# ingonyama-zk/icicle-snark

Measured on AMD Instinct MI355X. Metric: groth16_prove_constraints_per_s, higher is better.
Workload: dtype u256 mod p (MSM: 9x29-bit limbs in u32, Montgomery R=2^261, lazy reduction; NTT: 9x29-bit limbs, lazy; QAP/vec ops: 8xu32 limbs, Montgomery R=2^256)

## Files before the change

### icicle-snark_amd/csrc/ntt.hip

```cpp
#include <atomic>
#include <mutex>
#include <string.h>
#include <vector>

#include "common.h"
#include "ff.h"
#include "fr29.h"
#include "ntt_fuse.h"

using namespace bn254;
using namespace isnark;

namespace {

constexpr int LOG_TILE = 11;
constexpr int NT = 256;
constexpr int MAX_LOG_R = 9;
constexpr int OMEGAS_COUNT = 28;

const uint32_t ROU28[8] = {0x725b19f0, 0x9bd61b6e, 0x41112ed4, 0x402d111e, 0x8ef62abc, 0x00e0a7eb, 0xa58a7e85, 0x2a3c09f0};

struct Domain {
  fe* tw = nullptr;
  fe* tw29 = nullptr;
  int log_n = -1;
  fe root_std;
  int device = -1;
};
constexpr int MAX_DEVICES = 32;
std::mutex g_dom_mu;
Domain g_doms[MAX_DEVICES];
Domain& cur_dom()
{
  int d = 0;
  if (hipGetDevice(&d) != hipSuccess || d < 0 || d >= MAX_DEVICES) d = 0;
  return g_doms[d];
}
#define g_dom cur_dom()

fe host_omega(int logn)
{
  fe w;
  memcpy(w.l, ROU28, 32);
  w = Fr::to_mont(w);
  for (int i = 0; i < OMEGAS_COUNT - logn; i++) w = Fr::sqr(w);
  return Fr::from_mont(w);
}

__global__ void gen_twiddles_kernel(fe* tw, const fe* pw , int log_n)
{
  uint32_t i = blockIdx.x * blockDim.x + threadIdx.x;
  if (i >= (1u << log_n)) return;
  fe acc = Fr::one_mont();
  for (int j = 0; j < log_n; j++)
    if ((i >> j) & 1) acc = Fr::mul(acc, pw[j]);
  tw[i] = acc;
}

struct PassParams {
  int log_r, log_c;
  uint32_t tiles_per_group_log;
  uint64_t in_hi, in_lo, in_row, in_col;
  uint64_t out_hi, out_lo, out_row, out_col;
  uint32_t tw_mul;
  uint32_t stage_stride;
  uint32_t n_mask;
  int inverse;
  int scale;
  uint64_t batch_stride;
  int load_rows_fastest;
  const fe* scale_tab;
  uint32_t scale_stride;
  int fuse_abc;
  uint32_t xcd_batch;
};

__device__ __forceinline__ uint32_t tw_index(uint32_t e, uint32_t n_mask, int inverse)
{
  return inverse ? ((n_mask + 1 - e) & n_mask) : e;
}

__device__ __forceinline__ fe lds_get(const uint4* lo, const uint4* hi, int idx)
{
  uint4 a = lo[idx], b = hi[idx];
  fe r;
  r.l[0] = a.x; r.l[1] = a.y; r.l[2] = a.z; r.l[3] = a.w;
  r.l[4] = b.x; r.l[5] = b.y; r.l[6] = b.z; r.l[7] = b.w;
  return r;
}
__device__ __forceinline__ void lds_put(uint4* lo, uint4* hi, int idx, const fe& v)
{
  lo[idx] = make_uint4(v.l[0], v.l[1], v.l[2], v.l[3]);
  hi[idx] = make_uint4(v.l[4], v.l[5], v.l[6], v.l[7]);
}
__device__ __forceinline__ fe g_get(const fe* p)
{
  const uint4* q = reinterpret_cast<const uint4*>(p);
  uint4 a = q[0], b = q[1];
  fe r;
  r.l[0] = a.x; r.l[1] = a.y; r.l[2] = a.z; r.l[3] = a.w;
  r.l[4] = b.x; r.l[5] = b.y; r.l[6] = b.z; r.l[7] = b.w;
  return r;
}
__device__ __forceinline__ void g_put(fe* p, const fe& v)
{
  uint4* q = reinterpret_cast<uint4*>(p);
  q[0] = make_uint4(v.l[0], v.l[1], v.l[2], v.l[3]);
  q[1] = make_uint4(v.l[4], v.l[5], v.l[6], v.l[7]);
}

#define NTT_BF(a, b, e)                                                                                        \
  {                                                                                                            \
    const fe s_ = Fr::add(x[a], x[b]);                                                                         \
    const fe d_ = Fr::sub(x[a], x[b]);                                                                         \
    x[a] = s_;                                                                                                 \
    x[b] = Fr::mul(d_, lds_get(twlo, twhi, (e)));                                                              \
  }
template <int Q>
__device__ __forceinline__ void dif_butterfly(fe (&x)[1 << Q], int j, int log_m, int log_r, const uint4* twlo, const uint4* twhi);

template <>
__device__ __forceinline__ void dif_butterfly<3>(fe (&x)[8], int j, int log_m, int log_r, const uint4* twlo, const uint4* twhi)
{
  const int g = 1 << (log_m - 3);
  const int s0 = log_r - log_m, s1 = s0 + 1, s2 = s0 + 2;
  NTT_BF(0, 4, j << s0) NTT_BF(1, 5, (j + g) << s0) NTT_BF(2, 6, (j + 2 * g) << s0) NTT_BF(3, 7, (j + 3 * g) << s0)
  NTT_BF(0, 2, j << s1) NTT_BF(1, 3, (j + g) << s1) NTT_BF(4, 6, j << s1) NTT_BF(5, 7, (j + g) << s1)
  NTT_BF(0, 1, j << s2) NTT_BF(2, 3, j << s2) NTT_BF(4, 5, j << s2) NTT_BF(6, 7, j << s2)
}
template <>
__device__ __forceinline__ void dif_butterfly<2>(fe (&x)[4], int j, int log_m, int log_r, const uint4* twlo, const uint4* twhi)
{
  const int g = 1 << (log_m - 2);
  const int s0 = log_r - log_m, s1 = s0 + 1;
  NTT_BF(0, 2, j << s0) NTT_BF(1, 3, (j + g) << s0)
  NTT_BF(0, 1, j << s1) NTT_BF(2, 3, j << s1)
}
template <>
__device__ __forceinline__ void dif_butterfly<1>(fe (&x)[2], int j, int log_m, int log_r, const uint4* twlo, const uint4* twhi)
{
  NTT_BF(0, 1, j << (log_r - log_m))
}
#define NTT_BF1(a, b)                                                                                          \
  {                                                                                                            \
    const fe s_ = Fr::add(x[a], x[b]);                                                                         \
    x[b] = Fr::sub(x[a], x[b]);                                                                                \
    x[a] = s_;                                                                                                 \
  }
template <int Q>
__device__ __forceinline__ void dif_butterfly_last(fe (&x)[1 << Q], int log_r, const uint4* twlo, const uint4* twhi);
template <>
__device__ __forceinline__ void dif_butterfly_last<3>(fe (&x)[8], int log_r, const uint4* twlo, const uint4* twhi)
{
  const int s0 = log_r - 3, s1 = s0 + 1;
  NTT_BF1(0, 4) NTT_BF(1, 5, 1 << s0) NTT_BF(2, 6, 2 << s0) NTT_BF(3, 7, 3 << s0)
  NTT_BF1(0, 2) NTT_BF(1, 3, 1 << s1) NTT_BF1(4, 6) NTT_BF(5, 7, 1 << s1)
  NTT_BF1(0, 1) NTT_BF1(2, 3) NTT_BF1(4, 5) NTT_BF1(6, 7)
}
template <>
__device__ __forceinline__ void dif_butterfly_last<2>(fe (&x)[4], int log_r, const uint4* twlo, const uint4* twhi)
{
  const int s0 = log_r - 2;
  NTT_BF1(0, 2) NTT_BF(1, 3, 1 << s0)
  NTT_BF1(0, 1) NTT_BF1(2, 3)
}
template <>
__device__ __forceinline__ void dif_butterfly_last<1>(fe (&x)[2], int log_r, const uint4* twlo, const uint4* twhi)
{
  NTT_BF1(0, 1)
}
#undef NTT_BF1
#undef NTT_BF

template <int Q, bool LAST = false>
__device__ __forceinline__ void dif_round(uint4* lo, uint4* hi, const uint4* twlo, const uint4* twhi, int log_m, int log_r, int log_c, int tid)
{
  const int C = 1 << log_c;
  const int log_g = log_m - Q;
#pragma unroll
  for (int u = 0; u < (8 >> Q); u++) {
    const int gi = tid * (8 >> Q) + u;
    const int c = gi & (C - 1);
    const int rest = gi >> log_c;
    const int j = rest & ((1 << log_g) - 1);
    const int blk = rest >> log_g;
    const int base_row = (blk << log_m) + j;
    fe x[1 << Q];
#pragma unroll
    for (int k = 0; k < (1 << Q); k++) x[k] = lds_get(lo, hi, ((base_row + (k << log_g)) << log_c) + c);
    if (LAST) dif_butterfly_last<Q>(x, log_r, twlo, twhi);
    else dif_butterfly<Q>(x, j, log_m, log_r, twlo, twhi);
#pragma unroll
    for (int k = 0; k < (1 << Q); k++) lds_put(lo, hi, ((base_row + (k << log_g)) << log_c) + c, x[k]);
  }
}

template <int MODE>
__device__ __forceinline__ void ntt_tile_row(const fe* __restrict__ src, fe* __restrict__ dst, const fe* __restrict__ tw, const PassParams& p, const fe& ninv_mont, uint4* lo, uint4* hi,
                                             const uint4* twlo, const uint4* twhi, uint32_t b_lo, uint64_t out_off, int tid)
{
  const int R = 1 << p.log_r, C = 1 << p.log_c, RC = R * C;
  if (RC == NT * 8) {
    fe v[8];
#pragma unroll
    for (int u = 0; u < 8; u++) {
      const int e = tid + u * NT;
      int r, c;
      if (p.load_rows_fastest) { r = e & (R - 1); c = e >> p.log_r; }
      else { c = e & (C - 1); r = e >> p.log_c; }
      v[u] = g_get(src + (uint64_t)r * p.in_row + (uint64_t)c * p.in_col);
    }
#pragma unroll
    for (int u = 0; u < 8; u++) {
      const int e = tid + u * NT;
      int r, c;
      if (p.load_rows_fastest) { r = e & (R - 1); c = e >> p.log_r; }
      else { c = e & (C - 1); r = e >> p.log_c; }
      lds_put(lo, hi, (r << p.log_c) + c, v[u]);
    }
  } else {
    for (int e = tid; e < RC; e += NT) {
      int r, c;
      if (p.load_rows_fastest) { r = e & (R - 1); c = e >> p.log_r; }
      else { c = e & (C - 1); r = e >> p.log_c; }
      lds_put(lo, hi, (r << p.log_c) + c, g_get(src + (uint64_t)r * p.in_row + (uint64_t)c * p.in_col));
    }
  }
  __syncthreads();

  if (RC == NT * 8) {
    int log_m = p.log_r;
    while (log_m > 3) {
      dif_round<3>(lo, hi, twlo, twhi, log_m, p.log_r, p.log_c, tid);
      __syncthreads();
      log_m -= 3;
    }
    if (log_m == 3) dif_round<3, true>(lo, hi, twlo, twhi, log_m, p.log_r, p.log_c, tid);
    else if (log_m == 2) dif_round<2, true>(lo, hi, twlo, twhi, log_m, p.log_r, p.log_c, tid);
    else if (log_m == 1) dif_round<1, true>(lo, hi, twlo, twhi, log_m, p.log_r, p.log_c, tid);
    __syncthreads();
  } else {
    const int nbf = RC >> 1;
    for (int s = p.log_r - 1; s >= 0; s--) {
      const int h = 1 << s;
      for (int q = tid; q < nbf; q += NT) {
        const int c = q & (C - 1);
        const int bf = q >> p.log_c;
        const int j = bf & (h - 1);
        const int i = ((bf >> s) << (s + 1)) + j;
        const int ia = (i << p.log_c) + c, ib = ((i + h) << p.log_c) + c;
        fe a = lds_get(lo, hi, ia), bb = lds_get(lo, hi, ib);
        fe sum = Fr::add(a, bb);
        fe dif = Fr::sub(a, bb);
        const int e = j << (p.log_r - 1 - s);
        if (e != 0) dif = Fr::mul(dif, lds_get(twlo, twhi, e));
        lds_put(lo, hi, ia, sum);
        lds_put(lo, hi, ib, dif);
      }
      __syncthreads();
    }
  }

  if (MODE != 0) {
#pragma unroll 1
    for (int u0 = 0; u0 < 8; u0 += 4) {
      fe y[4];
      fe* q[4];
#pragma unroll
      for (int u = 0; u < 4; u++) {
        const int e = tid + (u0 + u) * NT;
        const int c = e & (C - 1);
        const uint32_t kk = __brev((uint32_t)(e >> p.log_c)) >> (32 - p.log_r);
        q[u] = dst + (uint64_t)kk * p.out_row + (uint64_t)c * p.out_col;
        if (MODE != 1) y[u] = g_get(q[u]);
      }
#pragma unroll
      for (int u = 0; u < 4; u++) {
        const fe x = lds_get(lo, hi, tid + (u0 + u) * NT);
        if (MODE == 1) g_put(q[u], x);
        else if (MODE == 2) g_put(q[u], Fr::mul(Fr::mul(x, y[u]), Fr::r2()));
        else g_put(q[u], Fr::sub(y[u], x));
      }
    }
    return;
  }
  for (int e0 = tid; e0 < RC; e0 += NT * 4) {
    fe w[4];
    uint32_t kk[4], ex[4];
#pragma unroll
    for (int u = 0; u < 4; u++) {
      const int e = e0 + u * NT;
      ex[u] = 0;
      if (e < RC) {
        const int c = e & (C - 1);
        kk[u] = __brev((uint32_t)(e >> p.log_c)) >> (32 - p.log_r);
        if (p.tw_mul) ex[u] = kk[u] * ((b_lo << p.log_c) + c) * p.tw_mul;
        if (ex[u]) w[u] = g_get(tw + tw_index(ex[u], p.n_mask, p.inverse));
      }
    }
#pragma unroll
    for (int u = 0; u < 4; u++) {
      const int e = e0 + u * NT;
      if (e < RC) {
        const int c = e & (C - 1);
        fe x = lds_get(lo, hi, e);
        if (ex[u]) x = Fr::mul(x, w[u]);
        if (p.scale_tab) x = Fr::mul(x, g_get(p.scale_tab + (out_off + (uint64_t)kk[u] * p.out_row + (uint64_t)c * p.out_col) * p.scale_stride));
        else if (p.scale) x = Fr::mul(x, ninv_mont);
        g_put(dst + (uint64_t)kk[u] * p.out_row + (uint64_t)c * p.out_col, x);
      }
    }
  }
}

template <bool FUSE>
__global__ __launch_bounds__(NT, 2) void ntt_pass_kernel(const fe* __restrict__ in, fe* __restrict__ out, const fe* __restrict__ tw, PassParams p, fe ninv_mont)
{
  ISNARK_CRITICAL_CHAIN_KERNEL();
  extern __shared__ __attribute__((aligned(16))) unsigned char smem[];
  const int R = 1 << p.log_r, C = 1 << p.log_c, RC = R * C;
  uint4* lo = reinterpret_cast<uint4*>(smem);
  uint4* hi = lo + RC;
  uint4* twlo = hi + RC;
  uint4* twhi = twlo + (R >> 1);

  const uint32_t b = blockIdx.x;
  const uint32_t b_hi = b >> p.tiles_per_group_log, b_lo = b & ((1u << p.tiles_per_group_log) - 1);
  const uint64_t in_off = b_hi * p.in_hi + b_lo * p.in_lo, out_off = b_hi * p.out_hi + b_lo * p.out_lo;
  const int tid = threadIdx.x;

  for (int e = tid; e < (R >> 1); e += NT) {
    fe w = g_get(tw + tw_index((uint32_t)e * p.stage_stride, p.n_mask, p.inverse));
    lds_put(twlo, twhi, e, w);
  }
  if (!FUSE) {
    ntt_tile_row<0>(in + (uint64_t)blockIdx.y * p.batch_stride + in_off, out + (uint64_t)blockIdx.y * p.batch_stride + out_off, tw, p, ninv_mont, lo, hi, twlo, twhi, b_lo, out_off, tid);
  } else {
    ntt_tile_row<1>(in + in_off, out + out_off, tw, p, ninv_mont, lo, hi, twlo, twhi, b_lo, out_off, tid);
    __syncthreads();
    ntt_tile_row<2>(in + p.batch_stride + in_off, out + out_off, tw, p, ninv_mont, lo, hi, twlo, twhi, b_lo, out_off, tid);
    __syncthreads();
    ntt_tile_row<3>(in + 2 * p.batch_stride + in_off, out + out_off, tw, p, ninv_mont, lo, hi, twlo, twhi, b_lo, out_off, tid);
  }
}

struct Plan29 {
  uint32_t b0;
  uint32_t bs;
  int shrink_last;
};
struct Lds29 {
  uint4 *lo, *hi;
  uint32_t* top;
};
__device__ __forceinline__ fe9 lds_get9(const Lds29& t, int idx)
{
  const uint4 a = t.lo[idx], b = t.hi[idx];
  fe9 r;
  r.l[0] = a.x; r.l[1] = a.y; r.l[2] = a.z; r.l[3] = a.w;
  r.l[4] = b.x; r.l[5] = b.y; r.l[6] = b.z; r.l[7] = b.w;
  r.l[8] = t.top[idx];
  return r;
}
__device__ __forceinline__ void lds_put9(const Lds29& t, int idx, const fe9& v)
{
  t.lo[idx] = make_uint4(v.l[0], v.l[1], v.l[2], v.l[3]);
  t.hi[idx] = make_uint4(v.l[4], v.l[5], v.l[6], v.l[7]);
  t.top[idx] = v.l[8];
}
__device__ __forceinline__ fe9 sub_k(const fe9& a, const fe9& b, const fr29::Limbs9& kc)
{
  fe9 o;
#pragma unroll
  for (int i = 0; i < 9; i++) o.l[i] = a.l[i] + (kc.v[i] - b.l[i]);
  return o;
}
#define NTT_BF9(a, b, e, NORM)                                                                                 \
  {                                                                                                            \
    const fe9 s_ = NORM ? fr29::norm(fr29::add(x[a], x[b])) : fr29::add(x[a], x[b]);                           \
    const fe9 d_ = sub_k(x[a], x[b], kc);                                                                      \
    x[a] = s_;                                                                                                 \
    x[b] = fr29::mul(d_, lds_get9(tw, (e)));                                                                   \
  }
#define NTT_BF9_1(a, b, NORM)                                                                                  \
  {                                                                                                            \
    const fe9 s_ = NORM ? fr29::norm(fr29::add(x[a], x[b])) : fr29::add(x[a], x[b]);                           \
    x[b] = fr29::norm(sub_k(x[a], x[b], kc));                                                                  \
    x[a] = s_;                                                                                                 \
  }
__device__ __forceinline__ uint32_t k_mid(const Plan29& pl, int l) { return (pl.b0 << l) + 1u; }
__device__ __forceinline__ uint32_t k_last(const Plan29& pl, int t) { return (pl.bs + 1u) << t; }

__device__ __forceinline__ void dif_butterfly9_mid(fe9 (&x)[8], int j, int log_m, int log_r, const Lds29& tw, const Plan29& pl)
{
  const int g = 1 << (log_m - 3);
  const int s0 = log_r - log_m, s1 = s0 + 1, s2 = s0 + 2;
  {
    const fr29::Limbs9 kc = fr29::kr_borrow_proof(k_mid(pl, s0), 1);
    NTT_BF9(0, 4, j << s0, false) NTT_BF9(1, 5, (j + g) << s0, false) NTT_BF9(2, 6, (j + 2 * g) << s0, false) NTT_BF9(3, 7, (j + 3 * g) << s0, false)
  }
  {
    const fr29::Limbs9 kc = fr29::kr_borrow_proof(k_mid(pl, s1), 2);
    NTT_BF9(0, 2, j << s1, true) NTT_BF9(1, 3, (j + g) << s1, true) NTT_BF9(4, 6, j << s1, true) NTT_BF9(5, 7, (j + g) << s1, true)
  }
  {
    const fr29::Limbs9 kc = fr29::kr_borrow_proof(k_mid(pl, s2), 1);
    NTT_BF9(0, 1, j << s2, true) NTT_BF9(2, 3, j << s2, true) NTT_BF9(4, 5, j << s2, true) NTT_BF9(6, 7, j << s2, true)
  }
}
template <int Q>
__device__ __forceinline__ void dif_butterfly9_last(fe9 (&x)[1 << Q], int log_r, const Lds29& tw, const Plan29& pl);
template <>
__device__ __forceinline__ void dif_butterfly9_last<3>(fe9 (&x)[8], int log_r, const Lds29& tw, const Plan29& pl)
{
  const int s0 = log_r - 3, s1 = s0 + 1;
  {
    const fr29::Limbs9 kc = fr29::kr_borrow_proof(k_last(pl, 0), 1);
    NTT_BF9_1(0, 4, false) NTT_BF9(1, 5, 1 << s0, false) NTT_BF9(2, 6, 2 << s0, false) NTT_BF9(3, 7, 3 << s0, false)
  }
  {
    const fr29::Limbs9 kc = fr29::kr_borrow_proof(k_last(pl, 1), 2);
    NTT_BF9_1(0, 2, true) NTT_BF9(1, 3, 1 << s1, true) NTT_BF9_1(4, 6, true) NTT_BF9(5, 7, 1 << s1, true)
  }
  {
    const fr29::Limbs9 kc = fr29::kr_borrow_proof(k_last(pl, 2), 1);
    NTT_BF9_1(0, 1, true) NTT_BF9_1(2, 3, true) NTT_BF9_1(4, 5, true) NTT_BF9_1(6, 7, true)
  }
}
template <>
__device__ __forceinline__ void dif_butterfly9_last<2>(fe9 (&x)[4], int log_r, const Lds29& tw, const Plan29& pl)
{
  const int s0 = log_r - 2;
  {
    const fr29::Limbs9 kc = fr29::kr_borrow_proof(k_last(pl, 0), 1);
    NTT_BF9_1(0, 2, false) NTT_BF9(1, 3, 1 << s0, false)
  }
  {
    const fr29::Limbs9 kc = fr29::kr_borrow_proof(k_last(pl, 1), 2);
    NTT_BF9_1(0, 1, true) NTT_BF9_1(2, 3, true)
  }
}
template <>
__device__ __forceinline__ void dif_butterfly9_last<1>(fe9 (&x)[2], int log_r, const Lds29& tw, const Plan29& pl)
{
  const fr29::Limbs9 kc = fr29::kr_borrow_proof(k_last(pl, 0), 1);
  NTT_BF9_1(0, 1, true)
}
#undef NTT_BF9_1
#undef NTT_BF9

template <int Q, bool LAST>
__device__ __forceinline__ void dif_round9(const Lds29& t, const Lds29& tw, int log_m, int log_r, int log_c, int tid, const Plan29& pl)
{
  const int C = 1 << log_c;
  const int log_g = log_m - Q;
#pragma unroll
  for (int u = 0; u < (8 >> Q); u++) {
    const int gi = tid * (8 >> Q) + u;
    const int c = gi & (C - 1);
    const int rest = gi >> log_c;
    const int j = rest & ((1 << log_g) - 1);
    const int blk = rest >> log_g;
    const int base_row = (blk << log_m) + j;
    fe9 x[1 << Q];
#pragma unroll
    for (int k = 0; k < (1 << Q); k++) x[k] = lds_get9(t, ((base_row + (k << log_g)) << log_c) + c);
    if constexpr (LAST) {
      if (pl.shrink_last) {
#pragma unroll
        for (int k = 0; k < (1 << Q); k++) x[k] = fr29::shrink(x[k]);
      }
      dif_butterfly9_last<Q>(x, log_r, tw, pl);
    } else dif_butterfly9_mid(x, j, log_m, log_r, tw, pl);
#pragma unroll
    for (int k = 0; k < (1 << Q); k++) lds_put9(t, ((base_row + (k << log_g)) << log_c) + c, x[k]);
  }
}

__device__ __forceinline__ fe9 shl5(const fe9& a)
{
  fe9 o;
  o.l[0] = (a.l[0] & 0xffffffu) << 5;
#pragma unroll
  for (int i = 1; i < 8; i++) o.l[i] = ((a.l[i] & 0xffffffu) << 5) | (a.l[i - 1] >> 24);
  o.l[8] = (a.l[8] << 5) | (a.l[7] >> 24);
  return o;
}

template <int MODE>
__device__ __forceinline__ void ntt_tile_row9(const fe* __restrict__ src, fe* __restrict__ dst, const fe* __restrict__ tw29, const PassParams& p, const Plan29& pl, const fe& ninv261, const Lds29& t,
                                              const Lds29& tw, uint32_t b_lo, uint64_t out_off, int tid)
{
  const int R = 1 << p.log_r, C = 1 << p.log_c;
  {
    fe v[8];
#pragma unroll
    for (int u = 0; u < 8; u++) {
      const int e = tid + u * NT;
      int r, c;
      if (p.load_rows_fastest) { r = e & (R - 1); c = e >> p.log_r; }
      else { c = e & (C - 1); r = e >> p.log_c; }
      v[u] = g_get(src + (uint64_t)r * p.in_row + (uint64_t)c * p.in_col);
    }
#pragma unroll
    for (int u = 0; u < 8; u++) {
      const int e = tid + u * NT;
      int r, c;
      if (p.load_rows_fastest) { r = e & (R - 1); c = e >> p.log_r; }
      else { c = e & (C - 1); r = e >> p.log_c; }
      lds_put9(t, (r << p.log_c) + c, fr29::unpack(v[u]));
    }
  }
  __syncthreads();
  {
    int log_m = p.log_r;
    while (log_m > 3) {
      dif_round9<3, false>(t, tw, log_m, p.log_r, p.log_c, tid, pl);
      __syncthreads();
      log_m -= 3;
    }
    if (log_m == 3) dif_round9<3, true>(t, tw, log_m, p.log_r, p.log_c, tid, pl);
    else if (log_m == 2) dif_round9<2, true>(t, tw, log_m, p.log_r, p.log_c, tid, pl);
    else dif_round9<1, true>(t, tw, log_m, p.log_r, p.log_c, tid, pl);
    __syncthreads();
  }
  if (MODE != 0) {
#pragma unroll 1
    for (int u0 = 0; u0 < 8; u0 += 4) {
      fe y[4];
      fe* q[4];
#pragma unroll
      for (int u = 0; u < 4; u++) {
        const int e = tid + (u0 + u) * NT;
        const int c = e & (C - 1);
        const uint32_t kk = __brev((uint32_t)(e >> p.log_c)) >> (32 - p.log_r);
        q[u] = dst + (uint64_t)kk * p.out_row + (uint64_t)c * p.out_col;
        if (MODE != 1) y[u] = g_get(q[u]);
      }
#pragma unroll
      for (int u = 0; u < 4; u++) {
        const fe9 x = lds_get9(t, tid + (u0 + u) * NT);
        if (MODE == 1) g_put(q[u], fr29::pack(fr29::canon(x)));
        else if (MODE == 2) g_put(q[u], fr29::pack(fr29::mul(fr29::mul(x, fr29::unpack(y[u])), fr29::r2())));
        else g_put(q[u], fr29::pack(fr29::canon(fr29::norm(fr29::sub<600>(fr29::unpack(y[u]), x)))));
      }
    }
    return;
  }
  for (int e0 = tid; e0 < NT * 8; e0 += NT * 4) {
    fe w[4];
    uint32_t kk[4];
#pragma unroll
    for (int u = 0; u < 4; u++) {
      const int e = e0 + u * NT;
      const int c = e & (C - 1);
      kk[u] = __brev((uint32_t)(e >> p.log_c)) >> (32 - p.log_r);
      if (p.tw_mul) w[u] = g_get(tw29 + tw_index(kk[u] * ((b_lo << p.log_c) + c) * p.tw_mul, p.n_mask, p.inverse));
      else if (p.scale_tab) w[u] = g_get(p.scale_tab + (out_off + (uint64_t)kk[u] * p.out_row + (uint64_t)c * p.out_col) * p.scale_stride);
    }
#pragma unroll
    for (int u = 0; u < 4; u++) {
      const int e = e0 + u * NT;
      const int c = e & (C - 1);
      fe9 x = lds_get9(t, e);
      if (p.tw_mul) x = fr29::mul(x, fr29::unpack(w[u]));
      else if (p.scale_tab) x = fr29::canon(shl5(fr29::mul(x, fr29::unpack(w[u]))));
      else if (p.scale) x = fr29::canon4(fr29::mul(x, fr29::unpack(ninv261)));
      else x = fr29::canon(x);
      g_put(dst + (uint64_t)kk[u] * p.out_row + (uint64_t)c * p.out_col, fr29::pack(x));
    }
  }
}

template <bool FUSE>
__global__ __launch_bounds__(NT, 2) void ntt_pass29_kernel(const fe* __restrict__ in, fe* __restrict__ out, const fe* __restrict__ tw29, PassParams p, Plan29 pl, fe ninv261)
{
  ISNARK_CRITICAL_CHAIN_KERNEL();
  extern __shared__ __attribute__((aligned(16))) unsigned char smem[];
  const int R = 1 << p.log_r, RC = NT * 8;
  Lds29 t, tw;
  t.lo = reinterpret_cast<uint4*>(smem);
  t.hi = t.lo + RC;
  tw.lo = t.hi + RC;
  tw.hi = tw.lo + (R >> 1);
  t.top = reinterpret_cast<uint32_t*>(tw.hi + (R >> 1));
  tw.top = t.top + RC;

  uint32_t b = blockIdx.x, row = blockIdx.y;
  if (!FUSE && p.xcd_batch) {
    const uint32_t w = b >> 3;
    row = w % p.xcd_batch;
    b = (w / p.xcd_batch) * 8 + (b & 7);
  }
  const uint32_t b_hi = b >> p.tiles_per_group_log, b_lo = b & ((1u << p.tiles_per_group_log) - 1);
  const uint64_t in_off = b_hi * p.in_hi + b_lo * p.in_lo, out_off = b_hi * p.out_hi + b_lo * p.out_lo;
  const int tid = threadIdx.x;
  for (int e = tid; e < (R >> 1); e += NT) lds_put9(tw, e, fr29::unpack(g_get(tw29 + tw_index((uint32_t)e * p.stage_stride, p.n_mask, p.inverse))));
  if (!FUSE) {
    ntt_tile_row9<0>(in + (uint64_t)row * p.batch_stride + in_off, out + (uint64_t)row * p.batch_stride + out_off, tw29, p, pl, ninv261, t, tw, b_lo, out_off, tid);
  } else {
    ntt_tile_row9<1>(in + in_off, out + out_off, tw29, p, pl, ninv261, t, tw, b_lo, out_off, tid);
    __syncthreads();
    ntt_tile_row9<2>(in + p.batch_stride + in_off, out + out_off, tw29, p, pl, ninv261, t, tw, b_lo, out_off, tid);
    __syncthreads();
    ntt_tile_row9<3>(in + 2 * p.batch_stride + in_off, out + out_off, tw29, p, pl, ninv261, t, tw, b_lo, out_off, tid);
  }
}

__global__ __launch_bounds__(256) void twiddles_to_261_kernel(const fe* __restrict__ tw, fe* __restrict__ tw29, uint64_t n)
{
  const uint64_t i = (uint64_t)blockIdx.x * blockDim.x + threadIdx.x;
  if (i < n) g_put(tw29 + i, fr29::pack(fr29::canon4(fr29::mul(fr29::unpack(g_get(tw + i)), fr29::c256_to_261()))));
}

__global__ __launch_bounds__(256) void relayout_kernel(const fe* __restrict__ in, fe* __restrict__ out, uint64_t n, int batch, int logn, int rev, int cols, int scatter)
{
  const uint64_t t = (uint64_t)blockIdx.x * blockDim.x + threadIdx.x;
  if (t >= n * (uint64_t)batch) return;
  const uint64_t b = t / n, i = t % n;
  const uint64_t j = rev ? (logn ? (uint64_t)(__brevll(i) >> (64 - logn)) : 0) : i;
  const uint64_t c = cols ? b + j * (uint64_t)batch : b * n + j;
  if (scatter) g_put(out + c, g_get(in + t));
  else g_put(out + t, g_get(in + c));
}

__global__ void coset_mul_kernel(fe* data, uint64_t n, int batch, const fe* gpow2 , int logn)
{
  uint64_t i = (uint64_t)blockIdx.x * blockDim.x + threadIdx.x;
  if (i >= n) return;
  fe acc = Fr::one_mont();
  for (int j = 0; j < logn; j++)
    if ((i >> j) & 1) acc = Fr::mul(acc, gpow2[j]);
  for (int b = 0; b < batch; b++) {
    fe v = g_get(data + (uint64_t)b * n + i);
    g_put(data + (uint64_t)b * n + i, Fr::mul(v, acc));
  }
}

int ilog2(uint64_t x)
{
  int l = 0;
  while ((1ull << l) < x) l++;
  return l;
}

}

namespace isnark {
const fe* ntt_domain_table(int* log_n)
{
  std::lock_guard<std::mutex> lk(g_dom_mu);
  if (log_n) *log_n = g_dom.log_n;
  return g_dom.tw;
}
}

ISNARK_API eIcicleError bn254_get_root_of_unity(uint64_t max_size, bn254_scalar_t* rou)
{
  if (!rou) return ICICLE_INVALID_POINTER;
  const int logn = ilog2(max_size);
  if (logn > OMEGAS_COUNT) {
    set_last_error("no root-of-unity of order 2^%d in the BN254 scalar field", logn);
    return ICICLE_INVALID_ARGUMENT;
  }
  fe w;
  if (logn == 0) w = Fr::one_std();
  else w = host_omega(logn);
  memcpy(rou->limbs, w.l, 32);
  return ICICLE_SUCCESS;
}

ISNARK_API eIcicleError bn254_ntt_init_domain(const bn254_scalar_t* primitive_root, const NTTInitDomainConfig* cfg)
{
  if (!primitive_root || !cfg) return ICICLE_INVALID_POINTER;
  ICICLE_TRY(require_device());
  std::lock_guard<std::mutex> lk(g_dom_mu);
  if (g_dom.tw) return ICICLE_SUCCESS;
  fe root;
  memcpy(root.l, primitive_root->limbs, 32);
  fe rm = Fr::to_mont(root);
  std::vector<fe> pw;
  fe cur = rm;
  int k = 0;
  while (!Fr::eq(cur, Fr::one_mont())) {
    pw.push_back(cur);
    cur = Fr::sqr(cur);
    if (++k > OMEGAS_COUNT) {
      set_last_error("ntt_init_domain: not a 2^k-th root of unity (k <= %d)", OMEGAS_COUNT);
      return ICICLE_INVALID_ARGUMENT;
    }
  }
  hipStream_t s = (hipStream_t)cfg->stream;
  const uint64_t N = 1ull << k;
  fe* tw = nullptr;
  fe* dpw = nullptr;
  HIP_TRY(hipMalloc(&tw, N * sizeof(fe)), ICICLE_ALLOCATION_FAILED);
  if (k > 0) {
    HIP_TRY(hipMalloc(&dpw, k * sizeof(fe)), ICICLE_ALLOCATION_FAILED);
    HIP_TRY(hipMemcpy(dpw, pw.data(), k * sizeof(fe), hipMemcpyHostToDevice), ICICLE_COPY_FAILED);
  }
  hipLaunchKernelGGL(gen_twiddles_kernel, dim3((unsigned)((N + 255) / 256)), dim3(256), 0, s, tw, dpw, k);
  ICICLE_TRY(check_launch("gen_twiddles"));
  HIP_TRY(hipStreamSynchronize(s), ICICLE_SYNCHRONIZATION_FAILED);
  if (dpw) (void)hipFree(dpw);
  fe* tw29 = nullptr;
  if (hipMalloc(&tw29, N * sizeof(fe)) == hipSuccess) {
    hipLaunchKernelGGL(twiddles_to_261_kernel, dim3((unsigned)((N + 255) / 256)), dim3(256), 0, s, tw, tw29, N);
    ICICLE_TRY(check_launch("twiddles_to_261"));
    HIP_TRY(hipStreamSynchronize(s), ICICLE_SYNCHRONIZATION_FAILED);
  } else {
    (void)hipGetLastError();
    tw29 = nullptr;
  }
  g_dom.tw = tw;
  g_dom.tw29 = tw29;
  g_dom.log_n = k;
  g_dom.root_std = root;
  (void)hipGetDevice(&g_dom.device);
  return ICICLE_SUCCESS;
}

ISNARK_API eIcicleError bn254_ntt_release_domain(void)
{
  std::lock_guard<std::mutex> lk(g_dom_mu);
  if (g_dom.tw) {
    (void)hipDeviceSynchronize();
    (void)hipFree(g_dom.tw);
    if (g_dom.tw29) (void)hipFree(g_dom.tw29);
  }
  Domain& d = g_dom;
  d = Domain();
  return ICICLE_SUCCESS;
}

ISNARK_API eIcicleError bn254_get_root_of_unity_from_domain(uint64_t logn, bn254_scalar_t* rou)
{
  if (!rou) return ICICLE_INVALID_POINTER;
  std::lock_guard<std::mutex> lk(g_dom_mu);
  if (!g_dom.tw || (int)logn > g_dom.log_n) {
    set_last_error("get_root_of_unity_from_domain: domain not initialised or too small");
    return ICICLE_INVALID_ARGUMENT;
  }
  fe w = Fr::to_mont(g_dom.root_std);
  for (int i = 0; i < g_dom.log_n - (int)logn; i++) w = Fr::sqr(w);
  w = Fr::from_mont(w);
  memcpy(rou->limbs, w.l, 32);
  return ICICLE_SUCCESS;
}

namespace {
bool plan29(int logn, int& np, int (&lr)[3])
{
  int best = 1 << 30;
  auto full = [&](const int* l, int n) {
    uint64_t rem = 1ull << logn;
    for (int pi = 0; pi < n; pi++) {
      const uint64_t C = 1ull << (LOG_TILE - l[pi]);
      if (pi < n - 1) {
        const uint64_t tail = rem >> l[pi];
        if (C > tail) return false;
        rem = tail;
      } else if (C > (1ull << l[0])) return false;
    }
    return true;
  };
  for (int a = 8; a >= 4; a--)
    for (int b = 8; b >= 4; b--) {
      {
        const int l2[2] = {a, b};
        const int cost = (a + 2) / 3 + (b + 2) / 3;
        if (a + b == logn && cost < best && full(l2, 2)) { best = cost; np = 2; lr[0] = a; lr[1] = b; lr[2] = 0; }
      }
      for (int c = 8; c >= 4; c--) {
        const int l3[3] = {a, b, c};
        const int cost = (a + 2) / 3 + (b + 2) / 3 + (c + 2) / 3 + 1;
        if (a + b + c == logn && cost < best && full(l3, 3)) { best = cost; np = 3; lr[0] = a; lr[1] = b; lr[2] = c; }
      }
    }
  return best < (1 << 30);
}
bool bounds29(int log_r, uint32_t b_in, uint32_t limit, Plan29& pl)
{
  memset(&pl, 0, sizeof pl);
  const int q_last = log_r % 3 ? log_r % 3 : 3;
  pl.b0 = b_in;
  uint32_t B = b_in << (log_r - q_last);
  uint32_t e = B;
  for (int k = 0; k < q_last; k++) e = 2 * e + 1;
  if (e > limit) {
    pl.shrink_last = 1;
    B = B / 4 + 2;
  }
  pl.bs = B;
  for (int k = 0; k < q_last; k++) {
    if (2 * B + 1 >= 1350) return false;
    B = 2 * B + 1;
  }
  return B <= limit && (uint64_t)b_in << (log_r - q_last) < 650;
}
}

namespace {
eIcicleError ntt_impl(const bn254_scalar_t* input, int size, NTTDir dir, const NTTConfig* cfg, bn254_scalar_t* output, const isnark::NttFuse* fuse)
{
  if (!cfg || !input || !output) return ICICLE_INVALID_POINTER;
  if (size <= 0 || (size & (size - 1))) {
    set_last_error("ntt: size %d is not a power of two", size);
    return ICICLE_INVALID_ARGUMENT;
  }
  if ((int)cfg->ordering < (int)kNN || (int)cfg->ordering > (int)kMN) {
    set_last_error("ntt: unknown ordering %d", (int)cfg->ordering);
    return ICICLE_INVALID_ARGUMENT;
  }
  const bool rev_in = cfg->ordering == kRN || cfg->ordering == kRR || cfg->ordering == kMN;
  const bool rev_out = cfg->ordering == kNR || cfg->ordering == kRR || cfg->ordering == kNM;
  ICICLE_TRY(require_device());
  const int logn = ilog2((uint64_t)size);
  Domain dom;
  {
    std::lock_guard<std::mutex> lk(g_dom_mu);
    dom = g_dom;
  }
  if (!dom.tw || logn > dom.log_n) {
    set_last_error("ntt: size 2^%d exceeds the initialised domain (2^%d)", logn, dom.log_n);
    return ICICLE_INVALID_ARGUMENT;
  }
  const int batch = cfg->batch_size > 0 ? cfg->batch_size : 1;
  const uint64_t n = (uint64_t)size, total = n * batch;
  hipStream_t s = (hipStream_t)cfg->stream;
  const bool inverse = dir == kInverse;

  Staged sin, sout;
  ICICLE_TRY(sin.in(input, total * sizeof(fe), cfg->are_inputs_on_device, s));
  ICICLE_TRY(sout.out(output, total * sizeof(fe), cfg->are_outputs_on_device, s));
  const fe* d_in = sin.ptr<fe>();
  fe* d_final = sout.ptr<fe>();
  const bool cols = cfg->columns_batch && batch > 1;
  WsScoped<fe> pre_block, post_block;
  if (rev_in || cols) {
    HIP_TRY(pre_block.alloc(total, s), ICICLE_ALLOCATION_FAILED);
    hipLaunchKernelGGL(relayout_kernel, dim3((unsigned)((total + 255) / 256)), dim3(256), 0, s, d_in, pre_block.p, n, batch, logn, rev_in ? 1 : 0, cols ? 1 : 0, 0);
    ICICLE_TRY(check_launch("ntt_relayout_in"));
    d_in = pre_block.p;
  }
  fe* d_out = d_final;
  if (rev_out || cols) {
    HIP_TRY(post_block.alloc(total, s), ICICLE_ALLOCATION_FAILED);
    d_out = post_block.p;
  }

  fe g;
  memcpy(g.l, cfg->coset_gen.limbs, 32);
  const bool has_coset = !Fr::eq(g, Fr::one_std());
  fe* d_gpow = nullptr;
  if (has_coset) {
    fe gm = Fr::to_mont(g);
    if (inverse) gm = Fr::inv(gm);
    std::vector<fe> gp(logn > 0 ? logn : 1);
    fe cur = gm;
    for (int j = 0; j < logn; j++) { gp[j] = cur; cur = Fr::sqr(cur); }
    HIP_TRY(hipMalloc((void**)&d_gpow, gp.size() * sizeof(fe)), ICICLE_ALLOCATION_FAILED);
    HIP_TRY(hipMemcpy(d_gpow, gp.data(), gp.size() * sizeof(fe), hipMemcpyHostToDevice), ICICLE_COPY_FAILED);
  }

  int np, lr[3] = {0, 0, 0};
  if (logn <= MAX_LOG_R) { np = 1; lr[0] = logn; }
  else if (logn <= 2 * MAX_LOG_R) { np = 2; lr[0] = (logn + 1) / 2; lr[1] = logn / 2; }
  else { np = 3; lr[0] = MAX_LOG_R; lr[1] = (logn - MAX_LOG_R + 1) / 2; lr[2] = (logn - MAX_LOG_R) / 2; }
  static const bool allow29 = env_int("ICICLE_SNARK_NTT29", 1) != 0;
  int np29 = 0, lr29[3] = {0, 0, 0};
  const bool use29 = allow29 && dom.tw29 && plan29(logn, np29, lr29);
  if (use29) {
    np = np29;
    for (int k = 0; k < 3; k++) lr[k] = lr29[k];
  }

  fe* scratch = nullptr;
  WsScoped<fe> scratch_block;
  const bool need_pre_coset = has_coset && !inverse;
  if (np > 1 || need_pre_coset) {
    HIP_TRY(scratch_block.alloc(total, s), ICICLE_ALLOCATION_FAILED);
    scratch = scratch_block;
  }
  if (need_pre_coset) {
    HIP_TRY(hipMemcpyAsync(scratch, d_in, total * sizeof(fe), hipMemcpyDeviceToDevice, s), ICICLE_COPY_FAILED);
    hipLaunchKernelGGL(coset_mul_kernel, dim3((unsigned)((n + 255) / 256)), dim3(256), 0, s, scratch, n, batch, d_gpow, logn);
    ICICLE_TRY(check_launch("coset_mul"));
    d_in = scratch;
  }

  fe ninv = Fr::zero();
  ninv.l[0] = 1;
  if (inverse) {
    fe nn = Fr::zero();
    nn.l[0] = (uint32_t)n;
    ninv = Fr::inv(Fr::to_mont(nn));
  }
  const uint32_t N = 1u << dom.log_n;
  const uint32_t dom_stride = N >> logn;

  uint64_t rem = n;
  for (int pi = 0; pi < np; pi++) {
    PassParams p;
    memset(&p, 0, sizeof p);
    const bool last = pi == np - 1;
    p.log_r = lr[pi];
    const uint64_t R = 1ull << p.log_r;
    const uint64_t tail = rem / R;
    int log_c = LOG_TILE - p.log_r;
    p.inverse = inverse;
    p.scale = last && inverse;
    p.n_mask = N - 1;
    p.stage_stride = N >> p.log_r;
    p.batch_stride = n;
    const fe* src = pi == 0 ? d_in : scratch;
    fe* dst = last ? d_out : scratch;
    uint64_t tiles;
    if (!last) {
      if ((uint64_t)(1 << log_c) > tail) log_c = ilog2(tail);
      p.log_c = log_c;
      const uint64_t C = 1ull << log_c;
      const uint64_t tpg = tail / C;
      p.tiles_per_group_log = ilog2(tpg);
      p.in_hi = rem; p.in_lo = C; p.in_row = tail; p.in_col = 1;
      p.out_hi = rem; p.out_lo = C; p.out_row = tail; p.out_col = 1;
      p.tw_mul = (uint32_t)((uint64_t)dom_stride * (n / rem));
      p.load_rows_fastest = 0;
      tiles = (n / rem) * tpg;
    } else {
      const uint64_t R1 = np == 1 ? 1 : (1ull << lr[0]);
      if ((uint64_t)(1 << log_c) > R1) log_c = ilog2(R1);
      p.log_c = log_c;
      const uint64_t C = 1ull << log_c;
      const uint64_t mid = n / (R1 * R);
      const uint64_t tpg = R1 / C;
      p.tiles_per_group_log = ilog2(tpg);
      p.in_lo = C * (n / R1); p.in_hi = R; p.in_row = 1; p.in_col = n / R1;
      p.out_lo = C; p.out_hi = R1; p.out_row = R1 * mid; p.out_col = 1;
      p.tw_mul = 0;
      p.load_rows_fastest = 1;
      tiles = tpg * mid;
    }
    const size_t lds = ((size_t)2 << (p.log_r + p.log_c)) * 16 + (size_t)(R >> 1) * 32 + 32;
    static std::atomic<bool> lds_attr_set[MAX_DEVICES];
    const int devi = dom.device >= 0 && dom.device < MAX_DEVICES ? dom.device : 0;
    if (!lds_attr_set[devi].load(std::memory_order_acquire)) {
      HIP_TRY(hipFuncSetAttribute((const void*)ntt_pass_kernel<false>, hipFuncAttributeMaxDynamicSharedMemorySize, 160 * 1024), ICICLE_UNKNOWN_ERROR);
      HIP_TRY(hipFuncSetAttribute((const void*)ntt_pass_kernel<true>, hipFuncAttributeMaxDynamicSharedMemorySize, 160 * 1024), ICICLE_UNKNOWN_ERROR);
      lds_attr_set[devi].store(true, std::memory_order_release);
    }
    const bool full_tile = ((size_t)1 << (p.log_r + p.log_c)) == (size_t)NT * 8;
    if (last && fuse && fuse->scale_tab && inverse) {
      p.scale_tab = fuse->scale_tab;
      p.scale_stride = fuse->scale_stride;
    }
    Plan29 pl29;
    size_t lds29 = 0;
    fe ninv261 = ninv;
    if (use29) {
      const bool ends_in_product = !last || (inverse && true);
      if (!full_tile || !bounds29(p.log_r, pi == 0 ? 1u : 4u, ends_in_product ? 506u : 598u, pl29)) {
        set_last_error("ntt: internal error — no radix-2^29 bound plan for a %d-bit pass", p.log_r);
        return ICICLE_UNKNOWN_ERROR;
      }
      lds29 = (size_t)NT * 8 * 36 + (size_t)(R >> 1) * 36;
      static std::atomic<bool> lds29_attr_set[MAX_DEVICES];
      if (!lds29_attr_set[devi].load(std::memory_order_acquire)) {
        HIP_TRY(hipFuncSetAttribute((const void*)ntt_pass29_kernel<false>, hipFuncAttributeMaxDynamicSharedMemorySize, 160 * 1024), ICICLE_UNKNOWN_ERROR);
        HIP_TRY(hipFuncSetAttribute((const void*)ntt_pass29_kernel<true>, hipFuncAttributeMaxDynamicSharedMemorySize, 160 * 1024), ICICLE_UNKNOWN_ERROR);
        lds29_attr_set[devi].store(true, std::memory_order_release);
      }
      fe c32 = Fr::zero();
      c32.l[0] = 32;
      ninv261 = Fr::mul(ninv, Fr::to_mont(c32));
    }
    if (last && fuse && fuse->fused_out) {
      if (!full_tile || batch != 3 || inverse || rev_out || cols) {
        set_last_error("ntt: fused epilogue needs a forward batch-of-3 transform with full tiles");
        return ICICLE_INVALID_ARGUMENT;
      }
      p.fuse_abc = 1;
      if (use29) hipLaunchKernelGGL(ntt_pass29_kernel<true>, dim3((unsigned)tiles, 1), dim3(NT), lds29, s, src, fuse->fused_out, dom.tw29, p, pl29, ninv261);
      else hipLaunchKernelGGL(ntt_pass_kernel<true>, dim3((unsigned)tiles, 1), dim3(NT), lds, s, src, fuse->fused_out, dom.tw, p, ninv);
    } else if (use29) {
      if (batch > 1 && tiles % 8 == 0 && (uint64_t)tiles * (uint64_t)batch < (1ull << 31)) {
        p.xcd_batch = (uint32_t)batch;
        hipLaunchKernelGGL(ntt_pass29_kernel<false>, dim3((unsigned)(tiles * batch), 1), dim3(NT), lds29, s, src, dst, dom.tw29, p, pl29, ninv261);
      } else
        hipLaunchKernelGGL(ntt_pass29_kernel<false>, dim3((unsigned)tiles, (unsigned)batch), dim3(NT), lds29, s, src, dst, dom.tw29, p, pl29, ninv261);
    } else {
      hipLaunchKernelGGL(ntt_pass_kernel<false>, dim3((unsigned)tiles, (unsigned)batch), dim3(NT), lds, s, src, dst, dom.tw, p, ninv);
    }
    ICICLE_TRY(check_launch("ntt_pass"));
    rem = tail;
  }

  if (has_coset && inverse) {
    hipLaunchKernelGGL(coset_mul_kernel, dim3((unsigned)((n + 255) / 256)), dim3(256), 0, s, d_out, n, batch, d_gpow, logn);
    ICICLE_TRY(check_launch("coset_mul"));
  }
  if (rev_out || cols) {
    hipLaunchKernelGGL(relayout_kernel, dim3((unsigned)((total + 255) / 256)), dim3(256), 0, s, d_out, d_final, n, batch, logn, rev_out ? 1 : 0, cols ? 1 : 0, 1);
    ICICLE_TRY(check_launch("ntt_relayout_out"));
  }
  pre_block.release();
  post_block.release();
  scratch_block.release();
  if (d_gpow) {
    HIP_TRY(hipStreamSynchronize(s), ICICLE_SYNCHRONIZATION_FAILED);
    HIP_TRY(hipFree(d_gpow), ICICLE_DEALLOCATION_FAILED);
  }
  ICICLE_TRY(sout.finish());
  return end_call(s, cfg->is_async);
}
}

ISNARK_API eIcicleError bn254_ntt(const bn254_scalar_t* input, int size, NTTDir dir, const NTTConfig* cfg, bn254_scalar_t* output)
{
  return ntt_impl(input, size, dir, cfg, output, nullptr);
}

namespace isnark {
eIcicleError ntt_fused(fe* d_inout, uint32_t n, int batch, bool inverse, hipStream_t s, const NttFuse& fuse)
{
  NTTConfig nc;
  memset(&nc, 0, sizeof nc);
  nc.stream = s;
  nc.coset_gen.limbs[0] = 1;
  nc.batch_size = batch;
  nc.ordering = kNN;
  nc.are_inputs_on_device = nc.are_outputs_on_device = true;
  nc.is_async = true;
  return ntt_impl((const bn254_scalar_t*)d_inout, (int)n, inverse ? kInverse : kForward, &nc, (bn254_scalar_t*)d_inout, &fuse);
}
bool ntt_fusable(uint32_t n) { return n >= (1u << 12); }
__global__ __launch_bounds__(256) void ntt_scaled_keys_kernel(const fe* __restrict__ tw, uint32_t tw_stride, uint32_t n, fe ninv_mont, fe* __restrict__ tab)
{
  const uint32_t i = blockIdx.x * blockDim.x + threadIdx.x;
  if (i < n) g_put(tab + i, Fr::mul(g_get(tw + (size_t)i * tw_stride), ninv_mont));
}
eIcicleError ntt_build_scaled_keys(uint32_t n, fe* d_tab, hipStream_t s)
{
  int lg = 0;
  const fe* tw = ntt_domain_table(&lg);
  if (!tw || (1ull << lg) < 2ull * n) {
    set_last_error("ntt_build_scaled_keys: the domain must hold 2n = %llu roots", 2ull * n);
    return ICICLE_INVALID_ARGUMENT;
  }
  fe nn = Fr::zero();
  nn.l[0] = n;
  const fe ninv = Fr::inv(Fr::to_mont(nn));
  hipLaunchKernelGGL(ntt_scaled_keys_kernel, dim3((n + 255) / 256), dim3(256), 0, s, tw, (uint32_t)((1ull << lg) / (2ull * n)), n, ninv, d_tab);
  return check_launch("ntt_scaled_keys");
}
}

namespace isnark {
__global__ void module_warm_ntt_kernel() {}
void module_warm_ntt(hipStream_t s) { hipLaunchKernelGGL(module_warm_ntt_kernel, dim3(1), dim3(1), 0, s); }
}
```

Baseline: 102.6 million.

## Keep fused NTT intermediate products in registers instead of global round-trips

In the fused three-input NTT pass, the intermediate A*B product and its partner are now held in a per-thread register carry array instead of being written to and re-read from global memory between the three sub-NTTs. Only the final (A*B - C) result is stored. The three sub-NTTs now run in a non-unrolled loop over a runtime mode to limit code size, with asm barriers and sched_barrier hints that constrain scheduling and register pressure. The trade-off is higher register pressure from holding eight field elements across the loop, which may reduce occupancy or cause spills.

```diff
diff --git a/icicle-snark_amd/csrc/ntt.hip b/icicle-snark_amd/csrc/ntt.hip
--- a/icicle-snark_amd/csrc/ntt.hip
+++ b/icicle-snark_amd/csrc/ntt.hip
@@ -381,6 +381,7 @@
     const fe9 d_ = sub_k(x[a], x[b], kc);                                                                      \
     x[a] = s_;                                                                                                 \
     x[b] = fr29::mul(d_, lds_get9(tw, (e)));                                                                   \
+    if constexpr (TIGHT_) __builtin_amdgcn_sched_barrier(0);                                                   \
   }
 #define NTT_BF9_1(a, b, NORM)                                                                                  \
   {                                                                                                            \
@@ -391,8 +392,10 @@
 __device__ __forceinline__ uint32_t k_mid(const Plan29& pl, int l) { return (pl.b0 << l) + 1u; }
 __device__ __forceinline__ uint32_t k_last(const Plan29& pl, int t) { return (pl.bs + 1u) << t; }
 
+template <bool TIGHT>
 __device__ __forceinline__ void dif_butterfly9_mid(fe9 (&x)[8], int j, int log_m, int log_r, const Lds29& tw, const Plan29& pl)
 {
+  constexpr bool TIGHT_ = TIGHT;
   const int g = 1 << (log_m - 3);
   const int s0 = log_r - log_m, s1 = s0 + 1, s2 = s0 + 2;
   {
@@ -413,6 +416,7 @@
 template <>
 __device__ __forceinline__ void dif_butterfly9_last<3>(fe9 (&x)[8], int log_r, const Lds29& tw, const Plan29& pl)
 {
+  constexpr bool TIGHT_ = false;
   const int s0 = log_r - 3, s1 = s0 + 1;
   {
     const fr29::Limbs9 kc = fr29::kr_borrow_proof(k_last(pl, 0), 1);
@@ -430,6 +434,7 @@
 template <>
 __device__ __forceinline__ void dif_butterfly9_last<2>(fe9 (&x)[4], int log_r, const Lds29& tw, const Plan29& pl)
 {
+  constexpr bool TIGHT_ = false;
   const int s0 = log_r - 2;
   {
     const fr29::Limbs9 kc = fr29::kr_borrow_proof(k_last(pl, 0), 1);
@@ -443,13 +448,14 @@
 template <>
 __device__ __forceinline__ void dif_butterfly9_last<1>(fe9 (&x)[2], int log_r, const Lds29& tw, const Plan29& pl)
 {
+  constexpr bool TIGHT_ = false;
   const fr29::Limbs9 kc = fr29::kr_borrow_proof(k_last(pl, 0), 1);
   NTT_BF9_1(0, 1, true)
 }
 #undef NTT_BF9_1
 #undef NTT_BF9
 
-template <int Q, bool LAST>
+template <int Q, bool LAST, bool TIGHT = false>
 __device__ __forceinline__ void dif_round9(const Lds29& t, const Lds29& tw, int log_m, int log_r, int log_c, int tid, const Plan29& pl)
 {
   const int C = 1 << log_c;
@@ -471,7 +477,7 @@
         for (int k = 0; k < (1 << Q); k++) x[k] = fr29::shrink(x[k]);
       }
       dif_butterfly9_last<Q>(x, log_r, tw, pl);
-    } else dif_butterfly9_mid(x, j, log_m, log_r, tw, pl);
+    } else dif_butterfly9_mid<TIGHT>(x, j, log_m, log_r, tw, pl);
 #pragma unroll
     for (int k = 0; k < (1 << Q); k++) lds_put9(t, ((base_row + (k << log_g)) << log_c) + c, x[k]);
   }
@@ -487,11 +493,14 @@
   return o;
 }
 
-template <int MODE>
+template <bool FUSED>
 __device__ __forceinline__ void ntt_tile_row9(const fe* __restrict__ src, fe* __restrict__ dst, const fe* __restrict__ tw29, const PassParams& p, const Plan29& pl, const fe& ninv261, const Lds29& t,
-                                              const Lds29& tw, uint32_t b_lo, uint64_t out_off, int tid)
+                                              const Lds29& tw, uint32_t b_lo, uint64_t out_off, int tid, int mode, fe* __restrict__ carry)
 {
   const int R = 1 << p.log_r, C = 1 << p.log_c;
+#define NTT_FRESH_TID()                                                                                        \
+  if constexpr (FUSED) asm volatile("" : "+v"(tid))
+  NTT_FRESH_TID();
   {
     fe v[8];
 #pragma unroll
@@ -515,60 +524,68 @@
   {
     int log_m = p.log_r;
     while (log_m > 3) {
-      dif_round9<3, false>(t, tw, log_m, p.log_r, p.log_c, tid, pl);
+      NTT_FRESH_TID();
+      dif_round9<3, false, FUSED>(t, tw, log_m, p.log_r, p.log_c, tid, pl);
       __syncthreads();
       log_m -= 3;
     }
+    NTT_FRESH_TID();
     if (log_m == 3) dif_round9<3, true>(t, tw, log_m, p.log_r, p.log_c, tid, pl);
     else if (log_m == 2) dif_round9<2, true>(t, tw, log_m, p.log_r, p.log_c, tid, pl);
     else dif_round9<1, true>(t, tw, log_m, p.log_r, p.log_c, tid, pl);
     __syncthreads();
   }
-  if (MODE != 0) {
-#pragma unroll 1
-    for (int u0 = 0; u0 < 8; u0 += 4) {
-      fe y[4];
-      fe* q[4];
-#pragma unroll
-      for (int u = 0; u < 4; u++) {
-        const int e = tid + (u0 + u) * NT;
-        const int c = e & (C - 1);
-        const uint32_t kk = __brev((uint32_t)(e >> p.log_c)) >> (32 - p.log_r);
-        q[u] = dst + (uint64_t)kk * p.out_row + (uint64_t)c * p.out_col;
-        if (MODE != 1) y[u] = g_get(q[u]);
-      }
-#pragma unroll
-      for (int u = 0; u < 4; u++) {
-        const fe9 x = lds_get9(t, tid + (u0 + u) * NT);
-        if (MODE == 1) g_put(q[u], fr29::pack(fr29::canon(x)));
-        else if (MODE == 2) g_put(q[u], fr29::pack(fr29::mul(fr29::mul(x, fr29::unpack(y[u])), fr29::r2())));
-        else g_put(q[u], fr29::pack(fr29::canon(fr29::norm(fr29::sub<600>(fr29::unpack(y[u]), x)))));
-      }
+  NTT_FRESH_TID();
+#undef NTT_FRESH_TID
+  if constexpr (FUSED) {
+    if (mode == 1) {
+#define NTT_EPI9(u) carry[u] = fr29::pack(fr29::canon(lds_get9(t, tid + (u) * NT)));
+      NTT_EPI9(0) NTT_EPI9(1) NTT_EPI9(2) NTT_EPI9(3) NTT_EPI9(4) NTT_EPI9(5) NTT_EPI9(6) NTT_EPI9(7)
+#undef NTT_EPI9
+    } else if (mode == 2) {
+#define NTT_EPI9(u) carry[u] = fr29::pack(fr29::mul(fr29::mul(lds_get9(t, tid + (u) * NT), fr29::unpack(carry[u])), fr29::r2()));
+      NTT_EPI9(0) NTT_EPI9(1) NTT_EPI9(2) NTT_EPI9(3) NTT_EPI9(4) NTT_EPI9(5) NTT_EPI9(6) NTT_EPI9(7)
+#undef NTT_EPI9
+    } else {
+#define NTT_EPI9(u)                                                                                                                          \
+  {                                                                                                                                          \
+    const int e = tid + (u) * NT;                                                                                                            \
+    const int c = e & (C - 1);                                                                                                               \
+    const uint32_t kk = __brev((uint32_t)(e >> p.log_c)) >> (32 - p.log_r);                                                                  \
+    g_put(dst + (uint64_t)kk * p.out_row + (uint64_t)c * p.out_col,                                                                          \
+          fr29::pack(fr29::canon(fr29::norm(fr29::sub<600>(fr29::unpack(carry[u]), lds_get9(t, e))))));                                      \
+  }
+      NTT_EPI9(0) NTT_EPI9(1) NTT_EPI9(2) NTT_EPI9(3) NTT_EPI9(4) NTT_EPI9(5) NTT_EPI9(6) NTT_EPI9(7)
+#undef NTT_EPI9
     }
     return;
   }
   for (int e0 = tid; e0 < NT * 8; e0 += NT * 4) {
     fe w[4];
     uint32_t kk[4];
-#pragma unroll
-    for (int u = 0; u < 4; u++) {
-      const int e = e0 + u * NT;
-      const int c = e & (C - 1);
-      kk[u] = __brev((uint32_t)(e >> p.log_c)) >> (32 - p.log_r);
-      if (p.tw_mul) w[u] = g_get(tw29 + tw_index(kk[u] * ((b_lo << p.log_c) + c) * p.tw_mul, p.n_mask, p.inverse));
-      else if (p.scale_tab) w[u] = g_get(p.scale_tab + (out_off + (uint64_t)kk[u] * p.out_row + (uint64_t)c * p.out_col) * p.scale_stride);
-    }
-#pragma unroll
-    for (int u = 0; u < 4; u++) {
-      const int e = e0 + u * NT;
-      const int c = e & (C - 1);
-      fe9 x = lds_get9(t, e);
-      if (p.tw_mul) x = fr29::mul(x, fr29::unpack(w[u]));
-      else if (p.scale_tab) x = fr29::canon(shl5(fr29::mul(x, fr29::unpack(w[u]))));
-      else if (p.scale) x = fr29::canon4(fr29::mul(x, fr29::unpack(ninv261)));
-      else x = fr29::canon(x);
-      g_put(dst + (uint64_t)kk[u] * p.out_row + (uint64_t)c * p.out_col, fr29::pack(x));
-    }
+#define NTT_ST9_W(u)                                                                                                                         \
+  {                                                                                                                                          \
+    const int e = e0 + (u) * NT;                                                                                                             \
+    const int c = e & (C - 1);                                                                                                               \
+    kk[u] = __brev((uint32_t)(e >> p.log_c)) >> (32 - p.log_r);                                                                              \
+    if (p.tw_mul) w[u] = g_get(tw29 + tw_index(kk[u] * ((b_lo << p.log_c) + c) * p.tw_mul, p.n_mask, p.inverse));  \
+    else if (p.scale_tab) w[u] = g_get(p.scale_tab + (out_off + (uint64_t)kk[u] * p.out_row + (uint64_t)c * p.out_col) * p.scale_stride);    \
+  }
+#define NTT_ST9_X(u)                                                                                                                         \
+  {                                                                                                                                          \
+    const int e = e0 + (u) * NT;                                                                                                             \
+    const int c = e & (C - 1);                                                                                                               \
+    fe9 x = lds_get9(t, e);                                                                                                                  \
+    if (p.tw_mul) x = fr29::mul(x, fr29::unpack(w[u]));                                           \
+    else if (p.scale_tab) x = fr29::canon(shl5(fr29::mul(x, fr29::unpack(w[u]))));  \
+    else if (p.scale) x = fr29::canon4(fr29::mul(x, fr29::unpack(ninv261)));                                                                 \
+    else x = fr29::canon(x);                                                                                                                 \
+    g_put(dst + (uint64_t)kk[u] * p.out_row + (uint64_t)c * p.out_col, fr29::pack(x));                                                       \
+  }
+    NTT_ST9_W(0) NTT_ST9_W(1) NTT_ST9_W(2) NTT_ST9_W(3)
+    NTT_ST9_X(0) NTT_ST9_X(1) NTT_ST9_X(2) NTT_ST9_X(3)
+#undef NTT_ST9_X
+#undef NTT_ST9_W
   }
 }
 
@@ -597,13 +614,16 @@
   const int tid = threadIdx.x;
   for (int e = tid; e < (R >> 1); e += NT) lds_put9(tw, e, fr29::unpack(g_get(tw29 + tw_index((uint32_t)e * p.stage_stride, p.n_mask, p.inverse))));
   if (!FUSE) {
-    ntt_tile_row9<0>(in + (uint64_t)row * p.batch_stride + in_off, out + (uint64_t)row * p.batch_stride + out_off, tw29, p, pl, ninv261, t, tw, b_lo, out_off, tid);
+    ntt_tile_row9<false>(in + (uint64_t)row * p.batch_stride + in_off, out + (uint64_t)row * p.batch_stride + out_off, tw29, p, pl, ninv261, t, tw, b_lo, out_off, tid, 0, nullptr);
   } else {
-    ntt_tile_row9<1>(in + in_off, out + out_off, tw29, p, pl, ninv261, t, tw, b_lo, out_off, tid);
-    __syncthreads();
-    ntt_tile_row9<2>(in + p.batch_stride + in_off, out + out_off, tw29, p, pl, ninv261, t, tw, b_lo, out_off, tid);
-    __syncthreads();
-    ntt_tile_row9<3>(in + 2 * p.batch_stride + in_off, out + out_off, tw29, p, pl, ninv261, t, tw, b_lo, out_off, tid);
+    fe carry[8];
+#pragma unroll
+    for (int u = 0; u < 8; u++) carry[u] = Fr::zero();
+#pragma unroll 1
+    for (int mode = 1; mode <= 3; mode++) {
+      if (mode > 1) __syncthreads();
+      ntt_tile_row9<true>(in + (uint64_t)(mode - 1) * p.batch_stride + in_off, out + out_off, tw29, p, pl, ninv261, t, tw, b_lo, out_off, tid, mode, carry);
+    }
   }
 }
 
```

Result: slower. 101.6 million (-1.0%).
